# clawrim/gcn10

Hardware: AMD Instinct MI355X
Metric: CN Gpixels/sec (higher is better)
Workload: dtype u8

## Files before the change

### gcn10_amd/csrc/gcn10_deflate_fused.hip

```cpp
#include <hip/hip_runtime.h>

#include <cstdint>
#include <cstring>

#include "gcn10_deflate_internal.hpp"
#include "gcn10_gpu.h"
#include "gcn10_gpu_internal.hpp"

using gcn10::as_stream;
using gcn10::fail;
using gcn10::u32x4;
using gcn10::use_device;
using namespace gcn10_deflate;

namespace {

constexpr int kGroup = 6;

struct FusedJob {
    const uint8_t *esa;
    const uint8_t *hx;
    const int32_t *cj;
    const uint8_t *class_of;
    uint16_t *tok;
// ... 1296 lines not shown
            }
            const uint32_t at = (uint32_t)kMaxStream - 4u;
            o[at] = (uint8_t)(adler >> 24);
            o[at + 1] = (uint8_t)(adler >> 16);
            o[at + 2] = (uint8_t)(adler >> 8);
            o[at + 3] = (uint8_t)adler;
        }
        const uint8_t *val = class_val + job.sel[j] * 256;
        const uint32_t xc = (uint32_t)(t & 63) * 4u;
        for (int i = 0; i < kTile / 4; i++) {
            const int r = i * 4 + (t >> 6);
            const uint32_t c4 = class_pixels4(job, tx * kTile + xc, ty * kTile + (uint32_t)r, sh.class_of);
            uint8_t *dst = o + 2 + (r >> 7) * (5 + 32768) + 5 + (r & 127) * kTile + xc;
            dst[0] = val[c4 & 0xffu];
            dst[1] = val[(c4 >> 8) & 0xffu];
            dst[2] = val[(c4 >> 16) & 0xffu];
            dst[3] = val[c4 >> 24];
        }
    }
}

}

extern "C" {

int gcn10_gpu_deflate_fused_available(gcn10_gpu_ctx *ctx)
{
    return ctx && ctx->n_tables > 0 && ctx->n_classes > 0 ? 1 : 0;
}

int gcn10_gpu_deflate_fused_strip(gcn10_gpu_ctx *ctx, const uint8_t *esa, int W, int rows, const int32_t *cj,
                                  unsigned cond_mask, unsigned table_mask, uint8_t *arena_dev, size_t arena_cap,
                                  uint32_t *table_dev, unsigned long long *cursor_dev, gcn10_stream_t stream)
{
    int rc = use_device(ctx);
    if (rc)
        return rc;
    if (ctx->n_tables == 0)
        return fail(GCN10_E_STATE, "gcn10_gpu_deflate_fused_strip: call gcn10_gpu_set_tables first");
    if (ctx->n_classes == 0)
        return fail(GCN10_E_STATE, "gcn10_gpu_deflate_fused_strip: the lookup tables define more than 256 pixel "
                                   "classes; use gcn10_gpu_cn_strip + gcn10_gpu_deflate_strip");
    if (!ctx->d_hx || ctx->hx_W == 0 || (uint32_t)W != ctx->hx_W)
        return fail(GCN10_E_STATE, "gcn10_gpu_deflate_fused_strip: call gcn10_gpu_prepare_tile for W=%d first", W);
    if (W <= 0 || rows < 0 || cond_mask == 0 || (cond_mask & ~3u) || table_mask == 0 ||
        (table_mask >> ctx->n_tables))
        return fail(GCN10_E_INVAL, "gcn10_gpu_deflate_fused_strip: bad shape or masks");
    if (rows == 0)
        return GCN10_OK;
    if (!esa || !cj || !arena_dev || !table_dev || !cursor_dev)
        return fail(GCN10_E_INVAL, "gcn10_gpu_deflate_fused_strip: null pointer");
    if ((reinterpret_cast<uintptr_t>(arena_dev) & 15u) != 0)
        return fail(GCN10_E_INVAL, "gcn10_gpu_deflate_fused_strip: arena must be 16-byte aligned");

    FusedJob job;
    memset(&job, 0, sizeof job);
    job.esa = esa;
    job.hx = ctx->d_hx;
    job.cj = cj;
    job.class_of = ctx->d_class_of;
    job.hx_stride = ctx->hx_stride;
    job.hx_rows = ctx->hx_rows;
    job.seg_align = (uint32_t)ctx->arena_segment_align;
    for (int r = 0; r < GCN10_N_RASTERS; r++)
        if ((cond_mask >> (r / 9)) & 1u && (table_mask >> (r % 9)) & 1u)
            job.sel[job.n_sel++] = (uint8_t)r;
    job.t.arena = arena_dev;
    job.t.table = table_dev;
    job.t.cursor = cursor_dev;
    job.t.W = (uint32_t)W;
    job.t.rows = (uint32_t)rows;
    job.t.across = ((uint32_t)W + kTile - 1) / kTile;
    job.t.down = ((uint32_t)rows + kTile - 1) / kTile;
    if (arena_cap >= 0xfffffffeull)
        return fail(GCN10_E_INVAL, "tile encoder: an arena of %zu bytes does not fit 32-bit stream offsets "
                                   "(use fewer rows per strip)", arena_cap);
    job.t.arena_cap = arena_cap;
    const uint32_t positions = job.t.across * job.t.down;
    if ((uint64_t)positions * (uint64_t)(kMaxStream + kSlotAlign) >= 0xffffffffull)
        return fail(GCN10_E_INVAL, "tile encoder: %u tile positions in one strip (use fewer rows per strip)", positions);
    const uint64_t nblocks = (uint64_t)positions * job.n_sel;
    job.t.n_tiles = (uint32_t)nblocks;

    const size_t stats_bytes = ((size_t)nblocks * ((size_t)kHistWords * 4 + (size_t)kBookBytes) + 255) & ~(size_t)255;
    const size_t tok_bytes = (size_t)positions * kTokStride * sizeof(uint16_t);
    const size_t ntok_bytes = ((size_t)positions * sizeof(uint32_t) + 15) & ~(size_t)15;
    const size_t need = stats_bytes + tok_bytes + ntok_bytes + (size_t)nblocks * 8 + (size_t)job.n_sel * ((positions + 63u) / 64u) * 4;
    rc = gcn10::grow_workspace(&ctx->deflate_ws, &ctx->deflate_ws_cap, need);
    if (rc)
        return rc;
    job.t.hist = reinterpret_cast<uint32_t *>(ctx->deflate_ws);
    job.t.books = reinterpret_cast<uint8_t *>(ctx->deflate_ws) + (size_t)nblocks * kHistWords * 4;
    job.tok = reinterpret_cast<uint16_t *>(reinterpret_cast<uint8_t *>(ctx->deflate_ws) + stats_bytes);
    job.n_tok = reinterpret_cast<uint32_t *>(reinterpret_cast<uint8_t *>(ctx->deflate_ws) + stats_bytes + tok_bytes);
    job.t.sizes = table_dev;
    if (ctx->fused_emit != 0) {
        job.t.sizes = reinterpret_cast<uint32_t *>(reinterpret_cast<uint8_t *>(ctx->deflate_ws) + stats_bytes + tok_bytes + ntok_bytes);
        job.t.chunk_tot = job.t.sizes + (size_t)nblocks * 2;
        job.t.n_chunks = (positions + 63u) / 64u;
    }

    static_assert(sizeof(SharedFA) <= 80 * 1024, "two fused statistics workgroups per CU");
    static_assert(sizeof(SharedFA2) <= 80 * 1024, "two segment-parallel statistics workgroups (32 waves) per CU");
    static_assert(sizeof(SharedFC) <= 20 * 1024, "eight fused emit workgroups per CU");
    static_assert(sizeof(SharedFC2) <= 16 * 1024, "ten wave-independent emit workgroups per CU by LDS");
    if (!ctx->fused_ready) {
// ... 29 lines not shown
```

### gcn10_amd/csrc/gcn10_gpu.hip

```cpp

#include <hip/hip_runtime.h>
#include <unistd.h>
#include <hip/hip_ext.h>

#include <cstdarg>
#include <cstdint>
#include <cstdio>
#include <cstdlib>
#include <cstring>
#include <new>

#include "gcn10_gpu.h"
#include "gcn10_gpu_internal.hpp"

using gcn10::as_stream;
using gcn10::fail;
using gcn10::u32x4;
using gcn10::use_device;

namespace {

constexpr int kThreads = 256;
constexpr int kPxPerLane = 16;
constexpr int kChunk = kThreads * kPxPerLane;
// ... 355 lines not shown
            else {
                p.out[c * 9 + p.single_k][i] = lut[s * (uint32_t)kPlane1 + lc];
            }
        }
    }
}

__global__ __launch_bounds__(kThreads) void stream_copy_kernel(const u32x4 *in, u32x4 *out, uint32_t nvec,
                                                               uint32_t ntrips)
{
    uint32_t step, end;
    for (uint32_t trip = first_chunk(ntrips, step, end, true); trip < end; trip += step) {
        u32x4 v[2];
        uint32_t idx[2];
#pragma unroll
        for (int u = 0; u < 2; u++) {
            idx[u] = (trip * 2u + u) * (uint32_t)kThreads + threadIdx.x;
            v[u] = __builtin_nontemporal_load(in + (idx[u] < nvec ? idx[u] : 0u));
        }
#pragma unroll
        for (int u = 0; u < 2; u++)
            if (idx[u] < nvec)
                __builtin_nontemporal_store(v[u], out + idx[u]);
    }
}

__global__ __launch_bounds__(kThreads) void cn_strip_bytes(const StripParams p,
                                                           uint32_t cond_mask)
{
    __shared__ __attribute__((aligned(16))) uint8_t lut[kLut16Bytes];
    for (int i = threadIdx.x; i < kLut16Bytes; i += kThreads)
        lut[i] = p.lut[i];
    __syncthreads();

    const uint32_t stride = gridDim.x * blockDim.x;
    for (uint32_t i = blockIdx.x * blockDim.x + threadIdx.x; i < p.npix; i += stride) {
        const uint32_t y = i / p.W;
        const uint32_t x = i - y * p.W;
        const uint32_t lc = p.esa[i];
        const uint32_t cd = p.hx[(size_t)soil_row(p, y) * p.hx_stride + x];
        for (int c = 0; c < 2; c++) {
            if (!(cond_mask & (1u << c)))
                continue;
            const uint32_t s = (cd >> (4 * c)) & 0xfu;
            const uint8_t *row = lut + s * (uint32_t)kPlane16 + lc * 16u;
            for (int k = 0; k < 9; k++)
                if (p.table_mask & (1u << k))
                    p.out[c * 9 + k][i] = row[k];
        }
    }
}

constexpr uint32_t kExpandRows = 4;

template <bool VEC>
__global__ __launch_bounds__(kThreads) void expand_x_codes(const uint8_t *coarse,
                                                           uint32_t hsx, uint32_t hsy,
                                                           const int32_t *ci, uint32_t W,
                                                           uint8_t *hx, uint32_t hx_stride,
                                                           uint32_t *hx4, uint32_t *complex, uint32_t gen)
{
    const uint32_t x = (blockIdx.x * blockDim.x + threadIdx.x) * 16u;
    const uint32_t r0 = blockIdx.y * kExpandRows;
    if (x >= hx_stride || r0 >= hsy)
        return;
    const uint8_t pad = (uint8_t)(kInvalidPlane | (kInvalidPlane << 4));
    uint32_t cx[16];
    if (VEC && x + 16u <= W) {
        const u32x4 *civ = reinterpret_cast<const u32x4 *>(ci + x);
#pragma unroll
        for (int j = 0; j < 4; j++) {
            const u32x4 c4 = civ[j];
#pragma unroll
            for (int q = 0; q < 4; q++)
                cx[4 * j + q] = c4[q] < hsx ? c4[q] : hsx - 1u;
        }
    }
    else {
#pragma unroll
        for (int q = 0; q < 16; q++) {
            const uint32_t xx = x + q;
            const uint32_t c = xx < W ? (uint32_t)ci[xx] : 0u;
            cx[q] = xx < W ? (c < hsx ? c : hsx - 1u) : 0xffffffffu;
        }
    }
    const uint32_t c_lo = cx[0], c_hi = cx[15];
    const uint32_t r1 = r0 + kExpandRows < hsy ? r0 + kExpandRows : hsy;
    uint32_t split = 0;
    bool compact = true, in_set = true;
#pragma unroll
    for (int q = 0; q < 16; q++) {
        const bool lo = cx[q] == c_lo;
        in_set = in_set && (lo || cx[q] == c_hi);
        compact = compact && (lo ? split == (uint32_t)q : cx[q] == c_hi);
        split += lo && split == (uint32_t)q ? 1u : 0u;
    }
    const bool two = c_lo != 0xffffffffu && c_hi != 0xffffffffu && in_set;
    if (hx4 && x < W && !compact && *reinterpret_cast<volatile uint32_t *>(complex) != gen)
        *reinterpret_cast<volatile uint32_t *>(complex) = gen;
    for (uint32_t r = r0; r < r1; r++) {
        const uint8_t *row = coarse + (size_t)r * hsx;
        u32x4 o;
        if (two) {
            const uint32_t code_lo = soil_code(row[c_lo]), code_hi = soil_code(row[c_hi]);
#pragma unroll
            for (int j = 0; j < 4; j++) {
                uint32_t w = 0;
#pragma unroll
                for (int q = 0; q < 4; q++)
                    w |= (cx[4 * j + q] == c_lo ? code_lo : code_hi) << (8 * q);
                o[j] = w;
            }
        }
        else {
#pragma unroll
            for (int j = 0; j < 4; j++) {
                uint32_t w = 0;
#pragma unroll
                for (int q = 0; q < 4; q++) {
                    const uint32_t c = cx[4 * j + q];
                    const uint8_t code = c == 0xffffffffu ? pad : soil_code(row[c]);
                    w |= (uint32_t)code << (8 * q);
                }
                o[j] = w;
            }
        }
        __builtin_nontemporal_store(o, reinterpret_cast<u32x4 *>(hx + (size_t)r * hx_stride + x));
        if (hx4)
            __builtin_nontemporal_store(compact ? (o[0] & 0xffu) | ((o[3] >> 24) << 8) | (split << 16) : 0x00ff0000u,
                                        hx4 + (size_t)r * (hx_stride / 16u) + x / 16u);
    }
}

__global__ __launch_bounds__(kThreads) void resample_rows(const uint8_t *coarse,
                                                          uint32_t hsx,
                                                          const int32_t *ci,
                                                          const int32_t *cj, uint32_t W,
                                                          uint32_t rows, uint8_t *out)
{
    const size_t npix = (size_t)W * rows;
    const size_t stride = (size_t)gridDim.x * blockDim.x;
    for (size_t i = (size_t)blockIdx.x * blockDim.x + threadIdx.x; i < npix; i += stride) {
        const uint32_t y = (uint32_t)(i / W);
        const uint32_t x = (uint32_t)(i - (size_t)y * W);
        out[i] = coarse[(size_t)(uint32_t)cj[y] * hsx + (uint32_t)ci[x]];
    }
}

__device__ __forceinline__ uint8_t remap_soil(uint8_t h, bool drained)
{
    if (h >= 11 && h <= 14)
        return drained ? (uint8_t)4 : (uint8_t)(h - 10);
    return h;
}

__global__ __launch_bounds__(kThreads) void modify_hysogs_kernel(uint8_t *h, size_t npix,
                                                                 int drained,
                                                                 size_t head, size_t nvec)
{
    const size_t stride = (size_t)gridDim.x * blockDim.x;
    const size_t tid = (size_t)blockIdx.x * blockDim.x + threadIdx.x;
    u32x4 *body = reinterpret_cast<u32x4 *>(h + head);
    for (size_t v = tid; v < nvec; v += stride) {
        u32x4 in = body[v];
        u32x4 o;
#pragma unroll
        for (int j = 0; j < 4; j++) {
            uint32_t w = 0;
#pragma unroll
            for (int q = 0; q < 4; q++)
                w |= (uint32_t)remap_soil((uint8_t)(in[j] >> (8 * q)), drained != 0) << (8 * q);
            o[j] = w;
        }
        body[v] = o;
    }
    const size_t tail0 = head + nvec * 16;
    const size_t nscalar = head + (npix - tail0);
    for (size_t s = tid; s < nscalar; s += stride) {
        const size_t i = s < head ? s : tail0 + (s - head);
        h[i] = remap_soil(h[i], drained != 0);
    }
}

// ... 124 lines not shown

thread_local char g_err[512] = "";

int fail(int code, const char *fmt, ...)
{
    va_list ap;
    va_start(ap, fmt);
    vsnprintf(g_err, sizeof g_err, fmt, ap);
    va_end(ap);
    return code;
}

int use_device(gcn10_gpu_ctx *ctx)
{
    if (!ctx)
        return fail(GCN10_E_INVAL, "null context");
    HIP_TRY(hipSetDevice(ctx->device));
    return GCN10_OK;
}

hipStream_t as_stream(gcn10_gpu_ctx *ctx, gcn10_stream_t s)
{
    return s ? reinterpret_cast<hipStream_t>(s) : ctx->main_stream;
}

int grow_workspace(void **ws, size_t *cap, size_t need)
{
    if (need <= *cap)
        return GCN10_OK;
    HIP_TRY(hipDeviceSynchronize());
    if (*ws)
        HIP_TRY(hipFree(*ws));
    *ws = nullptr;
    *cap = 0;
    HIP_TRY(hipMalloc(ws, need));
    *cap = need;
    return GCN10_OK;
}

}

namespace {

uint32_t stream_grid(const gcn10_gpu_ctx *ctx, uint64_t nchunks, int blocks_per_cu = 0)
{
    uint64_t cap = (uint64_t)ctx->n_cus * (blocks_per_cu > 0 ? blocks_per_cu : ctx->grid_blocks_per_cu);
    cap -= cap % 8u;
    if (cap < 8)
        cap = 8;
    uint64_t g = nchunks < cap ? nchunks : cap;
    return (uint32_t)(g ? g : 1);
}

}

extern "C" {

int gcn10_gpu_abi_version(void)
{
    return GCN10_GPU_ABI_VERSION;
}

const char *gcn10_gpu_last_error(void)
{
    return gcn10::g_err;
}

int gcn10_gpu_device_count(void)
{
    int n = 0;
    if (hipGetDeviceCount(&n) != hipSuccess)
        return 0;
    return n;
}

int gcn10_gpu_init(int device, gcn10_gpu_ctx **out)
{
    if (!out)
        return fail(GCN10_E_INVAL, "gcn10_gpu_init: null out pointer");
    *out = nullptr;
    int n = 0;
    hipError_t e = hipGetDeviceCount(&n);
    if (e != hipSuccess || n <= 0)
        return fail(GCN10_E_NODEVICE, "no HIP device visible (%s); this engine has no CPU fallback",
                    e != hipSuccess ? hipGetErrorString(e) : "device count 0");
    if (device < 0 || device >= n)
        return fail(GCN10_E_INVAL, "device %d out of range (0..%d)", device, n - 1);
    HIP_TRY(hipSetDevice(device));
    hipDeviceProp_t prop;
    HIP_TRY(hipGetDeviceProperties(&prop, device));
    if (strncmp(prop.gcnArchName, "gfx950", 6) != 0)
        return fail(GCN10_E_NODEVICE, "device %d is %s; this library carries gfx950 code only",
                    device, prop.gcnArchName);

    gcn10_gpu_ctx *ctx = new (std::nothrow) gcn10_gpu_ctx();
    if (!ctx)
        return fail(GCN10_E_NOMEM, "context allocation failed");
    ctx->device = device;
    ctx->n_cus = prop.multiProcessorCount;
    hipError_t e2 = hipStreamCreateWithFlags(&ctx->main_stream, hipStreamNonBlocking);
    if (e2 == hipSuccess)
        e2 = hipMalloc(reinterpret_cast<void **>(&ctx->d_lut16), kLut16Bytes);
    if (e2 == hipSuccess)
        e2 = hipMalloc(reinterpret_cast<void **>(&ctx->d_lut1), GCN10_N_TABLES * kLut1Bytes);
    if (e2 != hipSuccess) {
        int rc = fail(GCN10_E_HIP, "context setup: %s", hipGetErrorString(e2));
        gcn10_gpu_destroy(ctx);
        return rc;
    }
    *out = ctx;
    return GCN10_OK;
}

void gcn10_gpu_destroy(gcn10_gpu_ctx *ctx)
{
    if (!ctx)
        return;
    (void)hipSetDevice(ctx->device);
    if (ctx->main_stream) {
        (void)hipStreamSynchronize(ctx->main_stream);
        (void)hipStreamDestroy(ctx->main_stream);
    }
    if (ctx->d_lut16)
        (void)hipFree(ctx->d_lut16);
    if (ctx->d_lut1)
        (void)hipFree(ctx->d_lut1);
    if (ctx->d_hx_alloc)
        (void)hipFree(ctx->d_hx_alloc);
    if (ctx->deflate_ws)
        (void)hipFree(ctx->deflate_ws);
    if (ctx->inflate_ws)
        (void)hipFree(ctx->inflate_ws);
    if (ctx->lzw_ws)
        (void)hipFree(ctx->lzw_ws);
    if (ctx->d_class_of)
        (void)hipFree(ctx->d_class_of);
    delete ctx;
}

int gcn10_gpu_device_info(gcn10_gpu_ctx *ctx, char *name, size_t cap, size_t *hbm_bytes)
{
    int rc = use_device(ctx);
    if (rc)
        return rc;
    hipDeviceProp_t prop;
    HIP_TRY(hipGetDeviceProperties(&prop, ctx->device));
    if (name && cap)
        snprintf(name, cap, "%s (%s)", prop.name[0] ? prop.name : "AMD GPU", prop.gcnArchName);
    if (hbm_bytes)
        *hbm_bytes = prop.totalGlobalMem;
    return prop.multiProcessorCount;
}

int gcn10_gpu_pci_bus_id(int device, char *buf, size_t cap)
{
    if (!buf || cap < 13)
        return fail(GCN10_E_INVAL, "gcn10_gpu_pci_bus_id: buffer too small");
    HIP_TRY(hipDeviceGetPCIBusId(buf, (int)cap, device));
    return GCN10_OK;
}


int gcn10_gpu_malloc(gcn10_gpu_ctx *ctx, size_t bytes, void **dptr)
{
    int rc = use_device(ctx);
    if (rc)
        return rc;
    if (!dptr)
        return fail(GCN10_E_INVAL, "gcn10_gpu_malloc: null out pointer");
    *dptr = nullptr;
    HIP_TRY(hipMalloc(dptr, bytes ? bytes : 1));
    return GCN10_OK;
}

int gcn10_gpu_free(gcn10_gpu_ctx *ctx, void *dptr)
{
    int rc = use_device(ctx);
    if (rc)
        return rc;
    if (dptr)
        HIP_TRY(hipFree(dptr));
// ... 301 lines not shown
    return GCN10_OK;
}

int gcn10_gpu_calculate_cn(gcn10_gpu_ctx *ctx, const uint8_t *esa, const uint8_t *hsg,
                           size_t npix, int table_index, uint8_t *out, gcn10_stream_t stream)
{
    int rc = use_device(ctx);
    if (rc)
        return rc;
    if (ctx->n_tables == 0)
        return fail(GCN10_E_STATE, "gcn10_gpu_calculate_cn: call gcn10_gpu_set_tables first");
    if (table_index < 0 || table_index >= ctx->n_tables)
        return fail(GCN10_E_INVAL, "gcn10_gpu_calculate_cn: table %d not loaded (have %d)",
                    table_index, ctx->n_tables);
    if (npix == 0)
        return GCN10_OK;
    if (!esa || !hsg || !out)
        return fail(GCN10_E_INVAL, "gcn10_gpu_calculate_cn: null pointer");
    const uint8_t *img = ctx->d_lut1 + (size_t)table_index * kLut1Bytes;
    const bool vec = aligned16(esa) && aligned16(hsg) && aligned16(out);
    const uint64_t work = vec ? (npix / 16 + 2 * kThreads - 1) / (2 * kThreads) + 1
                              : (npix + kThreads - 1) / kThreads;
    const uint32_t grid = stream_grid(ctx, work);
    if (vec)
        hipLaunchKernelGGL(calculate_cn_kernel<true>, dim3(grid), dim3(kThreads), 0,
                           as_stream(ctx, stream), esa, hsg, npix, img, out);
    else
        hipLaunchKernelGGL(calculate_cn_kernel<false>, dim3(grid), dim3(kThreads), 0,
                           as_stream(ctx, stream), esa, hsg, npix, img, out);
    HIP_TRY(hipGetLastError());
    return GCN10_OK;
}


int gcn10_gpu_prepare_tile(gcn10_gpu_ctx *ctx, const uint8_t *coarse, int hsx, int hsy,
                           const int32_t *ci, int W, gcn10_stream_t stream)
{
    int rc = use_device(ctx);
    if (rc)
        return rc;
    if (hsx <= 0 || hsy <= 0 || W <= 0)
        return fail(GCN10_E_INVAL, "gcn10_gpu_prepare_tile: bad shape W=%d soil=%dx%d", W, hsx, hsy);
    if (!coarse || !ci)
        return fail(GCN10_E_INVAL, "gcn10_gpu_prepare_tile: null pointer");
    const uint32_t stride = (((uint32_t)W + 15u) & ~15u) + 16u;
    const size_t need = (size_t)stride * (size_t)hsy;
    if (need > ctx->hx_capacity) {
        HIP_TRY(hipDeviceSynchronize());
        if (ctx->d_hx_alloc)
            HIP_TRY(hipFree(ctx->d_hx_alloc));
        ctx->d_hx_alloc = ctx->d_hx = nullptr;
        ctx->d_hx4 = ctx->d_hx4_complex = nullptr;
        ctx->hx4_ready = false;
        ctx->hx_capacity = 0;
        const size_t need16 = (need + 15) & ~(size_t)15;
        HIP_TRY(hipMalloc(reinterpret_cast<void **>(&ctx->d_hx_alloc), 16 + need16 + need16 / 4 + 16));
        ctx->d_hx = ctx->d_hx_alloc + 16;
        ctx->d_hx4 = reinterpret_cast<uint32_t *>(ctx->d_hx + need16);
        ctx->d_hx4_complex = reinterpret_cast<uint32_t *>(ctx->d_hx + need16 + need16 / 4);
        HIP_TRY(hipMemsetAsync(ctx->d_hx4_complex, 0, 4, as_stream(ctx, stream)));
        ctx->hx4_gen = 0;
        ctx->hx_capacity = need;
    }
    uint32_t *hx4 = ctx->compact_soil ? ctx->d_hx4 : nullptr;
    ctx->hx4_ready = hx4 != nullptr;
    if (hx4 && ++ctx->hx4_gen == 0u)
        ctx->hx4_gen = 1u;
    ctx->hx_stride = stride;
    ctx->hx_W = (uint32_t)W;
    ctx->hx_rows = (uint32_t)hsy;
    dim3 grid((stride / 16 + kThreads - 1) / kThreads, ((uint32_t)hsy + kExpandRows - 1) / kExpandRows);
    if (aligned16(ci))
        hipLaunchKernelGGL(expand_x_codes<true>, grid, dim3(kThreads), 0, as_stream(ctx, stream),
                           coarse, (uint32_t)hsx, (uint32_t)hsy, ci, (uint32_t)W, ctx->d_hx, stride, hx4,
                           ctx->d_hx4_complex, ctx->hx4_gen);
    else
        hipLaunchKernelGGL(expand_x_codes<false>, grid, dim3(kThreads), 0, as_stream(ctx, stream),
                           coarse, (uint32_t)hsx, (uint32_t)hsy, ci, (uint32_t)W, ctx->d_hx, stride, hx4,
                           ctx->d_hx4_complex, ctx->hx4_gen);
    HIP_TRY(hipGetLastError());
    return GCN10_OK;
}

int gcn10_gpu_cn_strip(gcn10_gpu_ctx *ctx, const uint8_t *esa, int W, int rows,
                       const int32_t *cj, unsigned cond_mask, unsigned table_mask,
                       uint8_t *const out[GCN10_N_RASTERS], gcn10_stream_t stream)
{
    int rc = use_device(ctx);
    if (rc)
        return rc;
    if (ctx->n_tables == 0)
        return fail(GCN10_E_STATE, "gcn10_gpu_cn_strip: call gcn10_gpu_set_tables first");
    if (!ctx->d_hx || ctx->hx_W == 0)
        return fail(GCN10_E_STATE, "gcn10_gpu_cn_strip: call gcn10_gpu_prepare_tile first");
    if (W <= 0 || rows < 0 || (uint32_t)W != ctx->hx_W)
        return fail(GCN10_E_INVAL, "gcn10_gpu_cn_strip: W=%d rows=%d does not match prepared tile W=%u",
                    W, rows, ctx->hx_W);
    if ((uint64_t)W * (uint64_t)rows > 0x7fffffffull)
        return fail(GCN10_E_INVAL, "gcn10_gpu_cn_strip: strip of %d x %d exceeds 2^31-1 pixels", W, rows);
    if (cond_mask == 0 || (cond_mask & ~3u))
        return fail(GCN10_E_INVAL, "gcn10_gpu_cn_strip: cond_mask 0x%x", cond_mask);
    if (table_mask == 0 || (table_mask >> ctx->n_tables))
        return fail(GCN10_E_INVAL, "gcn10_gpu_cn_strip: table_mask 0x%x with %d tables loaded",
                    table_mask, ctx->n_tables);
    if (rows == 0)
        return GCN10_OK;
    if (!esa || !cj || !out)
        return fail(GCN10_E_INVAL, "gcn10_gpu_cn_strip: null pointer");

    StripParams p;
    memset(&p, 0, sizeof p);
    bool all_aligned = aligned16(esa);
    for (int c = 0; c < 2; c++) {
        for (int k = 0; k < 9; k++) {
            const int r = c * 9 + k;
            if ((cond_mask & (1u << c)) && (table_mask & (1u << k))) {
                if (!out[r])
                    return fail(GCN10_E_INVAL, "gcn10_gpu_cn_strip: out[%d] is null but selected", r);
                p.out[r] = out[r];
                all_aligned = all_aligned && aligned16(out[r]);
            }
        }
    }
    p.esa = esa;
    p.hx = ctx->d_hx;
    p.cj = cj;
    p.W = (uint32_t)W;
    p.rows = (uint32_t)rows;
    p.npix = (uint32_t)((uint64_t)W * (uint64_t)rows);
    p.hx_stride = ctx->hx_stride;
    p.hx_rows = ctx->hx_rows;
    p.nchunks = (p.npix + kChunk - 1) / kChunk;
    p.table_mask = table_mask;
    hipStream_t s = as_stream(ctx, stream);

    p.xcd_slabs = (uint32_t)ctx->xcd_slabs;
    p.nvec16 = p.npix & ~15u;
    if (ctx->hx4_ready && ctx->compact_soil && (p.W & 15u) == 0u) {
        p.hx4 = ctx->d_hx4;
        p.hx4_complex = ctx->d_hx4_complex;
        p.hx4_stride = ctx->hx_stride / 16u;
        p.hx4_gen = ctx->hx4_gen;
    }
    if (p.npix < 16u || p.W < kMinVectorW)
        all_aligned = false;
    if (!all_aligned) {
        p.lut = ctx->d_lut16;
        const uint32_t g = stream_grid(ctx, ((uint64_t)p.npix + kThreads - 1) / kThreads);
        if (ctx->time_start && ctx->time_stop) {
            void *args[] = { &p, &cond_mask };
            HIP_TRY(hipExtLaunchKernel(reinterpret_cast<const void *>(cn_strip_bytes), dim3(g), dim3(kThreads), args, 0,
                                       s, ctx->time_start, ctx->time_stop, 0));
            ctx->time_start = ctx->time_stop = nullptr;
        }
        else {
            hipLaunchKernelGGL(cn_strip_bytes, dim3(g), dim3(kThreads), 0, s, p, cond_mask);
        }
        ctx->last_kernel = "cn_strip_bytes";
    }
    else {
        const bool single = popcount(table_mask) == 1;
        const bool all = table_mask == 0x1ffu;
        const int n_streams = popcount(cond_mask) * popcount(table_mask);
        const bool tuned = single && ctx->single.set;
        const int ilp = tuned ? ctx->single.ilp
                              : single ? ctx->ilp1 : (ctx->ilp16 > 0 ? ctx->ilp16 : (n_streams > 9 ? 1 : 2));
        const bool nt = ctx->nontemporal != 0;
        if (single) {
            p.single_k = (uint32_t)__builtin_ctz(table_mask);
            p.lut = ctx->d_lut1 + (size_t)p.single_k * kLut1Bytes;
        }
        else {
            p.lut = ctx->d_lut16;
        }
        const bool pf = (tuned ? ctx->single.prefetch : ctx->prefetch) != 0 && ilp <= 2;
        p.nchunks = (p.nchunks + (uint32_t)ilp - 1) / (uint32_t)ilp;
        const uint32_t grid = stream_grid(ctx, p.nchunks, tuned ? ctx->single.grid_blocks_per_cu : 0);
        if (tuned)
            p.xcd_slabs = (uint32_t)ctx->single.xcd_slabs;
        strip_kernel_t fn = pick_strip_kernel(single, cond_mask, all, ilp, nt, pf);
        if (!fn)
            return fail(GCN10_E_INVAL, "gcn10_gpu_cn_strip: no kernel for ilp=%d", ilp);
        if (ctx->time_start && ctx->time_stop) {
            void *args[] = { &p };
            HIP_TRY(hipExtLaunchKernel(reinterpret_cast<const void *>(fn), dim3(grid), dim3(kThreads), args, 0,
                                       s, ctx->time_start, ctx->time_stop, 0));
            ctx->time_start = ctx->time_stop = nullptr;
        }
        else {
            hipLaunchKernelGGL(fn, dim3(grid), dim3(kThreads), 0, s, p);
        }
        snprintf(ctx->kernel_name, sizeof ctx->kernel_name, "cn_strip_kernel<%d, %u, %s, %d, %s, %s>",
                 single ? 1 : 0, cond_mask, (all || single) ? "true" : "false", ilp, nt ? "true" : "false",
                 pf ? "true" : "false");
        ctx->last_kernel = ctx->kernel_name;
    }
    HIP_TRY(hipGetLastError());
    return GCN10_OK;
// ... 218 lines not shown
```

### gcn10_amd/csrc/gcn10_gpu_internal.hpp

```cpp
#ifndef GCN10_GPU_INTERNAL_HPP
#define GCN10_GPU_INTERNAL_HPP

#include <hip/hip_runtime.h>

#include <cstdint>

#include "gcn10_gpu.h"

namespace gcn10 {

int fail(int code, const char *fmt, ...) __attribute__((format(printf, 2, 3)));

#define HIP_TRY(expr)                                                                   \
    do {                                                                                \
        hipError_t e_ = (expr);                                                         \
        if (e_ != hipSuccess)                                                           \
            return gcn10::fail(e_ == hipErrorOutOfMemory ? GCN10_E_NOMEM : GCN10_E_HIP, \
                               "%s: %s", #expr, hipGetErrorString(e_));                 \
    } while (0)

int use_device(gcn10_gpu_ctx *ctx);
hipStream_t as_stream(gcn10_gpu_ctx *ctx, gcn10_stream_t s);
int grow_workspace(void **ws, size_t *cap, size_t need);

typedef uint32_t u32x4 __attribute__((ext_vector_type(4)));

__device__ __forceinline__ bool inflate_window_ok(uint32_t out_len, uint32_t chunk_w, uint32_t src_x, uint32_t src_y,
                                                  uint32_t copy_w, uint32_t copy_h, uint32_t slot_bytes)
{
    if (copy_w == 0 || copy_h == 0)
        return true;
    if (chunk_w == 0 || out_len > slot_bytes || src_x > chunk_w || copy_w > chunk_w - src_x)
        return false;
    const unsigned long long last = (unsigned long long)(src_y + copy_h - 1u) * chunk_w + src_x + copy_w;
    return (unsigned long long)src_y + copy_h <= 0xffffffffull && last <= out_len;
}

void launch_lzw_decode(const uint8_t *comp_dev, const gcn10_inflate_tile *tiles_dev, uint32_t n_tiles,
                       uint8_t *scratch, uint32_t slot_bytes, uint32_t *status_dev, hipStream_t stream);

constexpr int kClassCodes = 36;

}

struct gcn10_gpu_ctx {
    int device = -1;
    int n_cus = 0;
    hipStream_t main_stream = nullptr;
    uint8_t *d_lut16 = nullptr;
    uint8_t *d_lut1 = nullptr;
    int n_tables = 0;
    uint8_t *d_hx = nullptr;
    uint8_t *d_hx_alloc = nullptr;
    uint32_t *d_hx4 = nullptr;
    uint32_t *d_hx4_complex = nullptr;
    uint32_t hx4_gen = 0;
    bool hx4_ready = false;
    int compact_soil = 1;
    size_t hx_capacity = 0;
    uint32_t hx_stride = 0;
    uint32_t hx_W = 0;
    uint32_t hx_rows = 0;
    const char *last_kernel = "";
    char kernel_name[96] = "";
    int grid_blocks_per_cu = 16;
    int ilp16 = 0;
    int ilp1 = 2;
    int nontemporal = 1;
    int xcd_slabs = 1;
    int prefetch = 1;
    struct SingleShape {
        bool set = false;
        int xcd_slabs = 1, grid_blocks_per_cu = 8, ilp = 2, prefetch = 1;
    } single;
    hipEvent_t time_start = nullptr, time_stop = nullptr;
    uint8_t *d_class_of = nullptr;
    int n_classes = 0;
    int arena_segment_align = 4096;
    int deflate_wave_codes = 1;
    int fused_parse = 1;
    int fused_emit = 1;
    int event_sync_sleep_us = 0;
    bool fused_ready = false;
    bool codes_ready = false;
    bool deflate_ready = false;
    void *deflate_ws = nullptr;
    size_t deflate_ws_cap = 0;
    void *inflate_ws = nullptr;
    size_t inflate_ws_cap = 0;
    void *lzw_ws = nullptr;
    size_t lzw_ws_cap = 0;
};

#endif
```

### gcn10_amd/csrc/gcn10_overview.hip

```cpp
#include <hip/hip_runtime.h>

#include <cstdint>

#include "gcn10_gpu_internal.hpp"

using namespace gcn10;

namespace {

constexpr int kThreads = 256;
constexpr int kPlanes = 6;
constexpr int kPlane16 = 256 * 16 + 16;
constexpr int kLut16Bytes = kPlanes * kPlane16;
constexpr int kMaxLevels = 8;
constexpr int kL1Tile = 128;
constexpr uint32_t kL1Rows = 4;

__device__ __forceinline__ uint8_t avg_of(uint32_t s, uint32_t n)
{
    return n == 0 ? (uint8_t)GCN10_NODATA : (uint8_t)((2u * s + n) / (2u * n));
}

struct NearestParams {
    const uint8_t *src;
// ... 131 lines not shown
        cur = nxt;
        nxt = t;
        Wl = Wk;
        Hl = Hk;
        w = wk;
        h = hk;
        side = sidek;
    }
}

}

extern "C" {

int gcn10_gpu_overview_nearest(gcn10_gpu_ctx *ctx, const uint8_t *src, int W, int H, int level, uint8_t *dst,
                               gcn10_stream_t stream)
{
    int rc = use_device(ctx);
    if (rc)
        return rc;
    if (!src || !dst || W <= 0 || H <= 0 || level < 1 || level > 30)
        return fail(GCN10_E_INVAL, "gcn10_gpu_overview_nearest: bad arguments W=%d H=%d level=%d", W, H, level);
    NearestParams p;
    p.src = src;
    p.dst = dst;
    p.W = (uint32_t)W;
    p.H = (uint32_t)H;
    p.level = (uint32_t)level;
    p.Wk = (uint32_t)(((int64_t)W + (1ll << level) - 1) >> level);
    p.Hk = (uint32_t)(((int64_t)H + (1ll << level) - 1) >> level);
    dim3 grid((p.Wk + kThreads - 1) / kThreads, p.Hk);
    hipLaunchKernelGGL(overview_nearest_kernel, grid, dim3(kThreads), 0, as_stream(ctx, stream), p);
    HIP_TRY(hipGetLastError());
    return GCN10_OK;
}

int gcn10_gpu_overview_average(gcn10_gpu_ctx *ctx, const uint8_t *esa, int W, int H, int y0, int rows,
                               const int32_t *cj, unsigned cond_mask, unsigned table_mask, int n_levels,
                               uint8_t *const *levels, gcn10_stream_t stream)
{
    int rc = use_device(ctx);
    if (rc)
        return rc;
    if (ctx->n_tables == 0)
        return fail(GCN10_E_STATE, "gcn10_gpu_overview_average: call gcn10_gpu_set_tables first");
    if (!ctx->d_hx || (int)ctx->hx_W != W)
        return fail(GCN10_E_STATE, "gcn10_gpu_overview_average: prepare the block's tile (W=%d) first", W);
    if (!esa || !cj || !levels || W <= 0 || H <= 0 || n_levels < 1 || n_levels > kMaxLevels || y0 < 0 ||
        rows <= 0 || y0 % 256 != 0 || y0 + rows > H || (rows % 256 != 0 && y0 + rows != H))
        return fail(GCN10_E_INVAL, "gcn10_gpu_overview_average: bad strip y0=%d rows=%d of %dx%d, %d levels "
                    "(strips start and end on multiples of 256 rows, 1..8 levels)", y0, rows, W, H, n_levels);
    if (cond_mask == 0 || (cond_mask & ~3u) || table_mask == 0 || (table_mask >> ctx->n_tables) != 0)
        return fail(GCN10_E_INVAL, "gcn10_gpu_overview_average: bad masks cond=%#x table=%#x", cond_mask, table_mask);
    AvgParams p = {};
    p.esa = esa;
    p.cj = cj;
    p.lut16 = ctx->d_lut16;
    p.hx = ctx->d_hx;
    p.hx_stride = ctx->hx_stride;
    p.hx_rows = ctx->hx_rows;
    p.W = (uint32_t)W;
    p.H = (uint32_t)H;
    p.cond_mask = cond_mask;
    p.table_mask = table_mask;
    p.n_levels = (uint32_t)n_levels;
    int q = 0;
    for (int r = 0; r < GCN10_N_RASTERS; r++) {
        if (!((cond_mask >> (r / 9)) & 1u) || !((table_mask >> (r % 9)) & 1u))
            continue;
        for (int k = 0; k < n_levels; k++) {
            p.out[r][k] = levels[q * n_levels + k];
            if (!p.out[r][k])
                return fail(GCN10_E_INVAL, "gcn10_gpu_overview_average: level %d of raster %d is NULL", k + 1, r);
        }
        q++;
    }
    const uint32_t W1 = ((uint32_t)W + 1u) >> 1;
    p.y1_begin = (uint32_t)y0 / 2u;
    p.y1_end = ((uint32_t)(y0 + rows) + 1u) / 2u;
    hipStream_t s = as_stream(ctx, stream);
    dim3 grid1((W1 + kThreads - 1) / kThreads, (p.y1_end - p.y1_begin + kL1Rows - 1) / kL1Rows);
    hipLaunchKernelGGL(overview_avg_level1_kernel, grid1, dim3(kThreads), 0, s, p);
    HIP_TRY(hipGetLastError());
    if (n_levels >= 2) {
        const uint32_t ty0 = (uint32_t)y0 / 256u, ty1 = ((uint32_t)(y0 + rows) + 255u) / 256u;
        dim3 grid2((W1 + kL1Tile - 1) / kL1Tile, ty1 - ty0, GCN10_N_RASTERS);
        hipLaunchKernelGGL(overview_avg_deeper_kernel, grid2, dim3(kThreads), 0, s, p, ty0);
        HIP_TRY(hipGetLastError());
    }
    return GCN10_OK;
}

}
```

### gcn10_amd/csrc/gcn10_stats.hip

```cpp
#include <hip/hip_runtime.h>

#include <cstdint>

#include "gcn10_gpu_internal.hpp"

using namespace gcn10;

namespace {

constexpr int kThreads = 256;
constexpr uint32_t kPxPerLane = 16;
constexpr uint32_t kChunk = kThreads * kPxPerLane;
constexpr int kBins = GCN10_PAIR_HIST_BINS;
constexpr int kHistWords = GCN10_PAIR_HIST_SIZE;
constexpr uint32_t kRowsPerItem = 4;
constexpr int kGridPerCu = 4;

__host__ __device__ inline uint32_t code_bin(uint32_t code)
{
    const uint32_t d = code & 15u, u = code >> 4;
    const uint32_t b = d == u ? d : 5u + u;
    return b < (uint32_t)kBins ? b : (uint32_t)kBins - 1u;
}

// ... 93 lines not shown
        if (x0 + kPxPerLane <= p.W) {
            typedef u32x4 u32x4_u __attribute__((aligned(1)));
            u32x4 e[kRowsPerItem], s[kRowsPerItem];
#pragma unroll
            for (uint32_t j = 0; j < kRowsPerItem; j++) {
                e[j] = *reinterpret_cast<const u32x4_u *>(erow[j]);
                s[j] = *reinterpret_cast<const u32x4 *>(srow[j]);
            }
#pragma unroll
            for (uint32_t j = 0; j < kRowsPerItem; j++)
                if (j < ny)
                    count16(h, e[j], s[j]);
        }
        else {
            for (uint32_t j = 0; j < ny; j++)
                count_tail(h, erow[j], srow[j], p.W - x0);
        }
    }
    __syncthreads();
    for (uint32_t i = threadIdx.x; i < (uint32_t)kHistWords; i += kThreads)
        if (h[i])
            atomicAdd(&p.hist[i], (unsigned long long)h[i]);
}

}

extern "C" {

int gcn10_gpu_pair_histogram_codes(uint8_t codes[GCN10_PAIR_HIST_BINS])
{
    if (!codes)
        return fail(GCN10_E_INVAL, "gcn10_gpu_pair_histogram_codes: null pointer");
    for (int b = 0; b < kBins; b++)
        codes[b] = 0x55;
    for (uint32_t d = 0; d <= 5; d++)
        codes[code_bin(d | d << 4)] = (uint8_t)(d | d << 4);
    for (uint32_t u = 1; u <= 3; u++)
        codes[code_bin(4u | u << 4)] = (uint8_t)(4u | u << 4);
    return GCN10_PAIR_HIST_BINS;
}

int gcn10_gpu_pair_histogram(gcn10_gpu_ctx *ctx, const uint8_t *esa, int W, int rows, const int32_t *cj,
                             unsigned long long *hist_dev, gcn10_stream_t stream)
{
    int rc = use_device(ctx);
    if (rc)
        return rc;
    if (!ctx->d_hx || (int)ctx->hx_W != W)
        return fail(GCN10_E_STATE, "gcn10_gpu_pair_histogram: prepare the block's tile (W=%d) first", W);
    if (!esa || !cj || !hist_dev || W <= 0 || rows < 0)
        return fail(GCN10_E_INVAL, "gcn10_gpu_pair_histogram: bad arguments W=%d rows=%d", W, rows);
    if (rows == 0)
        return GCN10_OK;
    HistParams p = {};
    p.esa = esa;
    p.hx = ctx->d_hx;
    p.cj = cj;
    p.hist = hist_dev;
    p.W = (uint32_t)W;
    p.rows = (uint32_t)rows;
    p.hx_stride = ctx->hx_stride;
    p.hx_rows = ctx->hx_rows;
    p.per_row = ((uint32_t)W + kChunk - 1u) / kChunk;
    const uint64_t items = (uint64_t)((p.rows + kRowsPerItem - 1u) / kRowsPerItem) * p.per_row;
    const uint64_t cap = (uint64_t)(ctx->n_cus > 0 ? ctx->n_cus : 256) * kGridPerCu;
    const uint32_t grid = (uint32_t)(items < cap ? items : cap);
    hipLaunchKernelGGL(pair_histogram_kernel, dim3(grid), dim3(kThreads), 0, as_stream(ctx, stream), p);
    HIP_TRY(hipGetLastError());
    return GCN10_OK;
}

}
```

Baseline: 2889.

## Build compact soil words first and expand soil bytes lazily only when needed

Tile preparation now writes the compact per-16-pixel soil word buffer in a dedicated kernel. The full byte-per-pixel soil plane is produced only when some tile group turns out to be complex, or later on demand, by converting the words to bytes for consumers that need them (fused deflate, overview, histogram, unaligned CN path). This aims to skip writing the large byte plane when the CN kernel can run from the compact words alone. The cost is an extra conditional kernel, event-based cross-stream tracking, and more state that can go stale.

```diff
diff --git a/gcn10_amd/csrc/gcn10_deflate_fused.hip b/gcn10_amd/csrc/gcn10_deflate_fused.hip
--- a/gcn10_amd/csrc/gcn10_deflate_fused.hip
+++ b/gcn10_amd/csrc/gcn10_deflate_fused.hip
@@ -1372,6 +1372,8 @@
         return fail(GCN10_E_INVAL, "gcn10_gpu_deflate_fused_strip: null pointer");
     if ((reinterpret_cast<uintptr_t>(arena_dev) & 15u) != 0)
         return fail(GCN10_E_INVAL, "gcn10_gpu_deflate_fused_strip: arena must be 16-byte aligned");
+    if ((rc = gcn10::ensure_soil_bytes(ctx, as_stream(ctx, stream))) != 0)
+        return rc;
 
     FusedJob job;
     memset(&job, 0, sizeof job);
diff --git a/gcn10_amd/csrc/gcn10_gpu.hip b/gcn10_amd/csrc/gcn10_gpu.hip
--- a/gcn10_amd/csrc/gcn10_gpu.hip
+++ b/gcn10_amd/csrc/gcn10_gpu.hip
@@ -431,52 +431,92 @@
 }
 
 constexpr uint32_t kExpandRows = 4;
+constexpr uint32_t kWordRows = 8;
+constexpr uint32_t kCondExpandBlocksPerCu = 2;
 
 template <bool VEC>
-__global__ __launch_bounds__(kThreads) void expand_x_codes(const uint8_t *coarse,
-                                                           uint32_t hsx, uint32_t hsy,
-                                                           const int32_t *ci, uint32_t W,
-                                                           uint8_t *hx, uint32_t hx_stride,
-                                                           uint32_t *hx4, uint32_t *complex, uint32_t gen)
+__device__ __forceinline__ void group_columns(const int32_t *ci, uint32_t x, uint32_t W, uint32_t hsx,
+                                              uint32_t (&cx)[16])
+{
+    if (VEC && x + 16u <= W) {
+        const u32x4 *civ = reinterpret_cast<const u32x4 *>(ci + x);
+#pragma unroll
+        for (int j = 0; j < 4; j++) {
+            const u32x4 c4 = civ[j];
+#pragma unroll
+            for (int q = 0; q < 4; q++)
+                cx[4 * j + q] = c4[q] < hsx ? c4[q] : hsx - 1u;
+        }
+    }
+    else {
+#pragma unroll
+        for (int q = 0; q < 16; q++) {
+            const uint32_t xx = x + q;
+            const uint32_t c = xx < W ? (uint32_t)ci[xx] : 0u;
+            cx[q] = xx < W ? (c < hsx ? c : hsx - 1u) : 0xffffffffu;
+        }
+    }
+}
+
+template <bool VEC>
+__global__ __launch_bounds__(kThreads) void soil_words(const uint8_t *__restrict__ coarse, uint32_t hsx, uint32_t hsy,
+                                                       const int32_t *__restrict__ ci, uint32_t W, uint32_t hx_stride,
+                                                       uint32_t *__restrict__ hx4, uint32_t *complex, uint32_t gen)
 {
     const uint32_t x = (blockIdx.x * blockDim.x + threadIdx.x) * 16u;
-    const uint32_t r0 = blockIdx.y * kExpandRows;
+    const uint32_t r0 = blockIdx.y * kWordRows;
+    if (x >= hx_stride || r0 >= hsy)
+        return;
+    uint32_t cx[16];
+    group_columns<VEC>(ci, x, W, hsx, cx);
+    const uint32_t c_lo = cx[0], c_hi = cx[15];
+    uint32_t split = 0;
+    bool compact = true;
+#pragma unroll
+    for (int q = 0; q < 16; q++) {
+        const bool lo = cx[q] == c_lo;
+        compact = compact && (lo ? split == (uint32_t)q : cx[q] == c_hi);
+        split += lo && split == (uint32_t)q ? 1u : 0u;
+    }
+    if (x < W && !compact && *reinterpret_cast<volatile uint32_t *>(complex) != gen)
+        *reinterpret_cast<volatile uint32_t *>(complex) = gen;
+    const uint32_t pad = (uint32_t)(kInvalidPlane | (kInvalidPlane << 4));
+    const bool pad_lo = c_lo == 0xffffffffu, pad_hi = c_hi == 0xffffffffu;
+    const uint8_t *col_lo = coarse + (pad_lo ? 0u : c_lo), *col_hi = coarse + (pad_hi ? 0u : c_hi);
+    uint32_t *out = hx4 + (size_t)r0 * (hx_stride / 16u) + x / 16u;
+    const uint32_t n = r0 + kWordRows < hsy ? kWordRows : hsy - r0;
+    uint8_t h_lo[kWordRows], h_hi[kWordRows];
+#pragma unroll
+    for (uint32_t k = 0; k < kWordRows; k++) {
+        const size_t at = (size_t)(k < n ? r0 + k : r0) * hsx;
+        h_lo[k] = col_lo[at];
+        h_hi[k] = col_hi[at];
+    }
+#pragma unroll
+    for (uint32_t k = 0; k < kWordRows; k++) {
+        const uint32_t a = pad_lo ? pad : soil_code(h_lo[k]), b = pad_hi ? pad : soil_code(h_hi[k]);
+        if (k < n)
+            __builtin_nontemporal_store(compact ? a | (b << 8) | (split << 16) : 0x00ff0000u,
+                                        out + (size_t)k * (hx_stride / 16u));
+    }
+}
+
+template <bool VEC>
+__device__ __forceinline__ void expand_rows(const uint8_t *coarse, uint32_t hsx, uint32_t hsy, const int32_t *ci,
+                                            uint32_t W, uint8_t *hx, uint32_t hx_stride, uint32_t x, uint32_t r0)
+{
     if (x >= hx_stride || r0 >= hsy)
         return;
     const uint8_t pad = (uint8_t)(kInvalidPlane | (kInvalidPlane << 4));
     uint32_t cx[16];
-    if (VEC && x + 16u <= W) {
-        const u32x4 *civ = reinterpret_cast<const u32x4 *>(ci + x);
-#pragma unroll
-        for (int j = 0; j < 4; j++) {
-            const u32x4 c4 = civ[j];
-#pragma unroll
-            for (int q = 0; q < 4; q++)
-                cx[4 * j + q] = c4[q] < hsx ? c4[q] : hsx - 1u;
-        }
-    }
-    else {
-#pragma unroll
-        for (int q = 0; q < 16; q++) {
-            const uint32_t xx = x + q;
-            const uint32_t c = xx < W ? (uint32_t)ci[xx] : 0u;
-            cx[q] = xx < W ? (c < hsx ? c : hsx - 1u) : 0xffffffffu;
-        }
-    }
+    group_columns<VEC>(ci, x, W, hsx, cx);
     const uint32_t c_lo = cx[0], c_hi = cx[15];
     const uint32_t r1 = r0 + kExpandRows < hsy ? r0 + kExpandRows : hsy;
-    uint32_t split = 0;
-    bool compact = true, in_set = true;
-#pragma unroll
-    for (int q = 0; q < 16; q++) {
-        const bool lo = cx[q] == c_lo;
-        in_set = in_set && (lo || cx[q] == c_hi);
-        compact = compact && (lo ? split == (uint32_t)q : cx[q] == c_hi);
-        split += lo && split == (uint32_t)q ? 1u : 0u;
-    }
+    bool in_set = true;
+#pragma unroll
+    for (int q = 0; q < 16; q++)
+        in_set = in_set && (cx[q] == c_lo || cx[q] == c_hi);
     const bool two = c_lo != 0xffffffffu && c_hi != 0xffffffffu && in_set;
-    if (hx4 && x < W && !compact && *reinterpret_cast<volatile uint32_t *>(complex) != gen)
-        *reinterpret_cast<volatile uint32_t *>(complex) = gen;
     for (uint32_t r = r0; r < r1; r++) {
         const uint8_t *row = coarse + (size_t)r * hsx;
         u32x4 o;
@@ -505,9 +545,47 @@
             }
         }
         __builtin_nontemporal_store(o, reinterpret_cast<u32x4 *>(hx + (size_t)r * hx_stride + x));
-        if (hx4)
-            __builtin_nontemporal_store(compact ? (o[0] & 0xffu) | ((o[3] >> 24) << 8) | (split << 16) : 0x00ff0000u,
-                                        hx4 + (size_t)r * (hx_stride / 16u) + x / 16u);
+    }
+}
+
+template <bool VEC>
+__global__ __launch_bounds__(kThreads) void expand_x_codes(const uint8_t *coarse,
+                                                           uint32_t hsx, uint32_t hsy,
+                                                           const int32_t *ci, uint32_t W,
+                                                           uint8_t *hx, uint32_t hx_stride,
+                                                           const uint32_t *only_if, uint32_t gen)
+{
+    if (only_if && (uint32_t)scalar_load_i32(reinterpret_cast<const int32_t *>(only_if), 0u) != gen)
+        return;
+    const uint32_t nbx = (hx_stride / 16u + blockDim.x - 1u) / blockDim.x;
+    const uint32_t items = nbx * ((hsy + kExpandRows - 1u) / kExpandRows);
+    for (uint32_t item = blockIdx.x; item < items; item += gridDim.x)
+        expand_rows<VEC>(coarse, hsx, hsy, ci, W, hx, hx_stride, ((item % nbx) * blockDim.x + threadIdx.x) * 16u,
+                         (item / nbx) * kExpandRows);
+}
+
+constexpr uint32_t kWordsPerTrip = 4;
+
+__global__ __launch_bounds__(kThreads) void words_to_bytes(const uint32_t *__restrict__ hx4, size_t nwords,
+                                                           uint8_t *__restrict__ hx, const uint32_t *complex,
+                                                           uint32_t gen)
+{
+    if ((uint32_t)scalar_load_i32(reinterpret_cast<const int32_t *>(complex), 0u) == gen)
+        return;
+    const size_t stride = (size_t)gridDim.x * blockDim.x * kWordsPerTrip;
+    for (size_t i0 = (size_t)blockIdx.x * blockDim.x * kWordsPerTrip + threadIdx.x; i0 < nwords; i0 += stride) {
+        uint32_t w[kWordsPerTrip];
+#pragma unroll
+        for (uint32_t u = 0; u < kWordsPerTrip; u++) {
+            const size_t i = i0 + (size_t)u * blockDim.x;
+            w[u] = hx4[i < nwords ? i : i0];
+        }
+#pragma unroll
+        for (uint32_t u = 0; u < kWordsPerTrip; u++) {
+            const size_t i = i0 + (size_t)u * blockDim.x;
+            if (i < nwords)
+                __builtin_nontemporal_store(expand_soil_word(w[u]), reinterpret_cast<u32x4 *>(hx + i * 16u));
+        }
     }
 }
 
@@ -738,6 +816,27 @@
     return (uint32_t)(g ? g : 1);
 }
 
+}
+
+int gcn10::ensure_soil_bytes(gcn10_gpu_ctx *ctx, hipStream_t stream)
+{
+    if (ctx->hx_bytes_gen == ctx->hx4_gen) {
+        if (ctx->hx_bytes_pending && stream != ctx->hx_bytes_stream)
+            HIP_TRY(hipStreamWaitEvent(stream, ctx->hx_bytes_event, 0));
+        return GCN10_OK;
+    }
+    if (!ctx->hx_bytes_event)
+        HIP_TRY(hipEventCreateWithFlags(&ctx->hx_bytes_event, hipEventDisableTiming));
+    const size_t nwords = (size_t)(ctx->hx_stride / 16u) * ctx->hx_rows;
+    const uint32_t grid = stream_grid(ctx, (nwords + kThreads * kWordsPerTrip - 1) / (kThreads * kWordsPerTrip), 8);
+    hipLaunchKernelGGL(words_to_bytes, dim3(grid), dim3(kThreads), 0, stream, ctx->d_hx4, nwords, ctx->d_hx,
+                       ctx->d_hx4_complex, ctx->hx4_gen);
+    HIP_TRY(hipGetLastError());
+    HIP_TRY(hipEventRecord(ctx->hx_bytes_event, stream));
+    ctx->hx_bytes_gen = ctx->hx4_gen;
+    ctx->hx_bytes_stream = stream;
+    ctx->hx_bytes_pending = true;
+    return GCN10_OK;
 }
 
 extern "C" {
@@ -813,6 +912,8 @@
         (void)hipFree(ctx->d_lut1);
     if (ctx->d_hx_alloc)
         (void)hipFree(ctx->d_hx_alloc);
+    if (ctx->hx_bytes_event)
+        (void)hipEventDestroy(ctx->hx_bytes_event);
     if (ctx->deflate_ws)
         (void)hipFree(ctx->deflate_ws);
     if (ctx->inflate_ws)
@@ -1220,6 +1321,8 @@
         ctx->d_hx_alloc = ctx->d_hx = nullptr;
         ctx->d_hx4 = ctx->d_hx4_complex = nullptr;
         ctx->hx4_ready = false;
+        ctx->hx_bytes_gen = 0;
+        ctx->hx_bytes_pending = false;
         ctx->hx_capacity = 0;
         const size_t need16 = (need + 15) & ~(size_t)15;
         HIP_TRY(hipMalloc(reinterpret_cast<void **>(&ctx->d_hx_alloc), 16 + need16 + need16 / 4 + 16));
@@ -1230,22 +1333,37 @@
         ctx->hx4_gen = 0;
         ctx->hx_capacity = need;
     }
-    uint32_t *hx4 = ctx->compact_soil ? ctx->d_hx4 : nullptr;
-    ctx->hx4_ready = hx4 != nullptr;
-    if (hx4 && ++ctx->hx4_gen == 0u)
+    hipStream_t s = as_stream(ctx, stream);
+    if (ctx->hx_bytes_pending && s != ctx->hx_bytes_stream)
+        HIP_TRY(hipStreamWaitEvent(s, ctx->hx_bytes_event, 0));
+    ctx->hx_bytes_pending = false;
+    ctx->hx4_ready = ctx->compact_soil != 0;
+    if (++ctx->hx4_gen == 0u)
         ctx->hx4_gen = 1u;
     ctx->hx_stride = stride;
     ctx->hx_W = (uint32_t)W;
     ctx->hx_rows = (uint32_t)hsy;
-    dim3 grid((stride / 16 + kThreads - 1) / kThreads, ((uint32_t)hsy + kExpandRows - 1) / kExpandRows);
-    if (aligned16(ci))
-        hipLaunchKernelGGL(expand_x_codes<true>, grid, dim3(kThreads), 0, as_stream(ctx, stream),
-                           coarse, (uint32_t)hsx, (uint32_t)hsy, ci, (uint32_t)W, ctx->d_hx, stride, hx4,
-                           ctx->d_hx4_complex, ctx->hx4_gen);
-    else
-        hipLaunchKernelGGL(expand_x_codes<false>, grid, dim3(kThreads), 0, as_stream(ctx, stream),
-                           coarse, (uint32_t)hsx, (uint32_t)hsy, ci, (uint32_t)W, ctx->d_hx, stride, hx4,
-                           ctx->d_hx4_complex, ctx->hx4_gen);
+    const bool vec = aligned16(ci);
+    const uint32_t nbx = (stride / 16 + kThreads - 1) / kThreads;
+    const uint32_t items = nbx * (((uint32_t)hsy + kExpandRows - 1) / kExpandRows);
+    uint32_t expand_grid = items;
+    const uint32_t *only_if = nullptr;
+    if (ctx->hx4_ready) {
+        dim3 grid(nbx, ((uint32_t)hsy + kWordRows - 1) / kWordRows);
+        hipLaunchKernelGGL(vec ? soil_words<true> : soil_words<false>, grid, dim3(kThreads), 0, s, coarse,
+                           (uint32_t)hsx, (uint32_t)hsy, ci, (uint32_t)W, stride, ctx->d_hx4, ctx->d_hx4_complex,
+                           ctx->hx4_gen);
+        HIP_TRY(hipGetLastError());
+        const uint32_t cap = (uint32_t)(ctx->n_cus > 0 ? ctx->n_cus : 256) * kCondExpandBlocksPerCu;
+        expand_grid = items < cap ? items : cap;
+        only_if = ctx->d_hx4_complex;
+    }
+    else {
+        ctx->hx_bytes_gen = ctx->hx4_gen;
+    }
+    hipLaunchKernelGGL(vec ? expand_x_codes<true> : expand_x_codes<false>, dim3(expand_grid), dim3(kThreads), 0, s,
+                       coarse, (uint32_t)hsx, (uint32_t)hsy, ci, (uint32_t)W, ctx->d_hx, stride, only_if,
+                       ctx->hx4_gen);
     HIP_TRY(hipGetLastError());
     return GCN10_OK;
 }
@@ -1312,6 +1430,11 @@
     }
     if (p.npix < 16u || p.W < kMinVectorW)
         all_aligned = false;
+    if (!p.hx4 || !all_aligned) {
+        rc = gcn10::ensure_soil_bytes(ctx, s);
+        if (rc)
+            return rc;
+    }
     if (!all_aligned) {
         p.lut = ctx->d_lut16;
         const uint32_t g = stream_grid(ctx, ((uint64_t)p.npix + kThreads - 1) / kThreads);
diff --git a/gcn10_amd/csrc/gcn10_gpu_internal.hpp b/gcn10_amd/csrc/gcn10_gpu_internal.hpp
--- a/gcn10_amd/csrc/gcn10_gpu_internal.hpp
+++ b/gcn10_amd/csrc/gcn10_gpu_internal.hpp
@@ -39,6 +39,8 @@
 void launch_lzw_decode(const uint8_t *comp_dev, const gcn10_inflate_tile *tiles_dev, uint32_t n_tiles,
                        uint8_t *scratch, uint32_t slot_bytes, uint32_t *status_dev, hipStream_t stream);
 
+int ensure_soil_bytes(gcn10_gpu_ctx *ctx, hipStream_t stream);
+
 constexpr int kClassCodes = 36;
 
 }
@@ -56,6 +58,10 @@
     uint32_t *d_hx4_complex = nullptr;
     uint32_t hx4_gen = 0;
     bool hx4_ready = false;
+    uint32_t hx_bytes_gen = 0;
+    hipStream_t hx_bytes_stream = nullptr;
+    hipEvent_t hx_bytes_event = nullptr;
+    bool hx_bytes_pending = false;
     int compact_soil = 1;
     size_t hx_capacity = 0;
     uint32_t hx_stride = 0;
diff --git a/gcn10_amd/csrc/gcn10_overview.hip b/gcn10_amd/csrc/gcn10_overview.hip
--- a/gcn10_amd/csrc/gcn10_overview.hip
+++ b/gcn10_amd/csrc/gcn10_overview.hip
@@ -207,6 +207,8 @@
                     "(strips start and end on multiples of 256 rows, 1..8 levels)", y0, rows, W, H, n_levels);
     if (cond_mask == 0 || (cond_mask & ~3u) || table_mask == 0 || (table_mask >> ctx->n_tables) != 0)
         return fail(GCN10_E_INVAL, "gcn10_gpu_overview_average: bad masks cond=%#x table=%#x", cond_mask, table_mask);
+    if ((rc = gcn10::ensure_soil_bytes(ctx, as_stream(ctx, stream))) != 0)
+        return rc;
     AvgParams p = {};
     p.esa = esa;
     p.cj = cj;
diff --git a/gcn10_amd/csrc/gcn10_stats.hip b/gcn10_amd/csrc/gcn10_stats.hip
--- a/gcn10_amd/csrc/gcn10_stats.hip
+++ b/gcn10_amd/csrc/gcn10_stats.hip
@@ -169,6 +169,8 @@
         return fail(GCN10_E_INVAL, "gcn10_gpu_pair_histogram: bad arguments W=%d rows=%d", W, rows);
     if (rows == 0)
         return GCN10_OK;
+    if ((rc = gcn10::ensure_soil_bytes(ctx, as_stream(ctx, stream))) != 0)
+        return rc;
     HistParams p = {};
     p.esa = esa;
     p.hx = ctx->d_hx;
```

Result: faster. 2940 (median of 6 runs) (+1.7%).
